# tiddoloos/Scaling-RGCN-training

Hardware: AMD Instinct MI355X
Metric: edges/s per RGCN layer (fwd+bwd) (higher is better)
Workload: dtype f32 (contraction: bf16x3 split of fp32 operands, fp32 accumulate)

## Files before the change

### include/rgcn_mi355x.h

```cpp
#ifndef RGCN_MI355X_H
#define RGCN_MI355X_H

#include <stddef.h>
#include <stdint.h>

#ifdef __cplusplus
extern "C" {
#endif

#define RGCN_ABI_VERSION 19
#define RGCN_UNIT 64
#define RGCN_CHUNK_MAX 128
#define RGCN_MAX_WIDTH 128
#define RGCN_XWIDE_MAX_WIDTH 512
#define RGCN_DW_WALKERS 2048

enum rgcn_act { RGCN_ACT_NONE = 0, RGCN_ACT_RELU = 1, RGCN_ACT_SIGMOID = 2 };

#define RGCN_FLAG_POINTER_GATHER 1u
#define RGCN_FLAG_DW_RING 2u
#define RGCN_FLAG_DW_DIRECT 4u
#define RGCN_FLAG_DW_ROOT_ONLY 16u
#define RGCN_FLAG_SPLIT_PRODUCERS 32u
#define RGCN_FLAG_EXACT_FP32 8u

enum rgcn_status {
    RGCN_OK = 0,
    RGCN_ERR_NULL = -1,
    RGCN_ERR_WIDTH = -2,
    RGCN_ERR_STRIDE = -3,
    RGCN_ERR_PLAN = -4,
    RGCN_ERR_LDS = -5,
    RGCN_ERR_WORKSPACE = -6,
    RGCN_ERR_DEVICE = -7,
    RGCN_ERR_ACT = -8,
    RGCN_ERR_GRAPH = -9,
    RGCN_ERR_ADDRESS = -10
};

typedef struct rgcn_plan {
    int32_t n_nodes;
    int32_t n_owned;
    int32_t num_relations;
    int32_t tile;
    int32_t n_tiles;
    int32_t n_chunks;
    int32_t chunk;
    int32_t n_units;
    int32_t layout;
    int32_t chunk_rows;
    const int32_t* tile_ptr;
    const int32_t* chunk_rel;
    const int32_t* chunk_cnt;
    const int32_t* chunk_tile;
    const int32_t* chunk_flags;
    const int32_t* rel_order;
    const int32_t* slot_src;
    const float* slot_w;
    const int32_t* slot_row;
    const int32_t* slot_acc;
    const int32_t* slot_src2;
} rgcn_plan_t;

int rgcn_abi_version(void);
const char* rgcn_status_string(int status);

typedef struct rgcn_graph {
    const int64_t* src;
    const int64_t* dst;
    const int64_t* type;
    int64_t src_stride, dst_stride, type_stride;
    int64_t num_edges;
    int32_t num_nodes;
    int32_t num_relations;
} rgcn_graph_t;

typedef struct rgcn_plan_sizes {
    int32_t n_tiles;
    int32_t n_chunks;
    int32_t n_units;
    int32_t reserved;
    int64_t n_slots;
    int64_t n_edges;
    uint64_t opaque[16];
} rgcn_plan_sizes_t;

size_t rgcn_plan_workspace_bytes(int64_t num_edges, int32_t n_owned, int32_t num_relations, int32_t tile);

int rgcn_edge_weights(const rgcn_graph_t* graph, int aggr_sum, float* w, void* workspace, size_t workspace_bytes, void* stream);

int rgcn_plan_build_begin(const rgcn_graph_t* graph, const float* w, int transposed, int32_t node_begin, int32_t node_end,
                          int32_t tile, int32_t chunk, int32_t layout, void* workspace, size_t workspace_bytes,
                          rgcn_plan_sizes_t* sizes, void* stream);
int rgcn_plan_build_finish(const rgcn_plan_sizes_t* sizes, void* workspace, size_t workspace_bytes, rgcn_plan_t* plan,
                           void* stream);

int rgcn_padded_width(int width);

size_t rgcn_packed_weight_floats(int num_relations, int din, int dout);

int rgcn_pack_weights(const float* weight, const float* root, int num_relations, int din, int dout,
                      int transpose, float* packed, void* stream);
int rgcn_pack_weights_basis(const float* bases, const float* comp, const float* root, int num_relations, int num_bases,
                            int din, int dout, int transpose, float* packed, void* stream);
int rgcn_pack_weights_block(const float* blocks, const float* root, int num_relations, int num_blocks, int din, int dout,
                            int transpose, float* packed, void* stream);
int rgcn_basis_backward(const float* d_w, const float* bases, const float* comp, int num_relations, int num_bases, int din,
// ... 81 lines not shown
```

### scaling_rgcn_training_amd/_lib.py

```python
from __future__ import annotations

import ctypes as C
import os
from typing import Optional

import torch

_HERE = os.path.dirname(os.path.abspath(__file__))
LIB_PATH = os.environ.get("RGCN_LIB") or os.path.join(_HERE, "librgcn_mi355x.so")
ABI_VERSION = 19

XWIDE_MAX_WIDTH = 512

ACT_NONE, ACT_RELU, ACT_SIGMOID = 0, 1, 2
ERR_PLAN = -4
ERR_ADDRESS = -10
FLAG_POINTER_GATHER, FLAG_DW_RING, FLAG_DW_DIRECT, FLAG_EXACT_FP32, FLAG_DW_ROOT_ONLY, FLAG_SPLIT_PRODUCERS = 1, 2, 4, 8, 16, 32


class RgcnPlanStruct(C.Structure):
    _fields_ = [
        ("n_nodes", C.c_int32), ("n_owned", C.c_int32), ("num_relations", C.c_int32),
        ("tile", C.c_int32), ("n_tiles", C.c_int32), ("n_chunks", C.c_int32), ("chunk", C.c_int32), ("n_units", C.c_int32),
        ("layout", C.c_int32), ("chunk_rows", C.c_int32),
        ("tile_ptr", C.c_void_p), ("chunk_rel", C.c_void_p), ("chunk_cnt", C.c_void_p),
        ("chunk_tile", C.c_void_p), ("chunk_flags", C.c_void_p), ("rel_order", C.c_void_p), ("slot_src", C.c_void_p),
        ("slot_w", C.c_void_p), ("slot_row", C.c_void_p), ("slot_acc", C.c_void_p), ("slot_src2", C.c_void_p),
    ]


class RgcnEdgeUnits(C.Structure):
    _fields_ = [("n_nodes", C.c_int32), ("n_units", C.c_int32), ("num_relations", C.c_int32), ("reserved", C.c_int32),
                ("unit_rel", C.c_void_p), ("unit_cnt", C.c_void_p), ("slot_src", C.c_void_p), ("slot_w", C.c_void_p)]


class RgcnGraphStruct(C.Structure):
    _fields_ = [("src", C.c_void_p), ("dst", C.c_void_p), ("type", C.c_void_p),
                ("src_stride", C.c_int64), ("dst_stride", C.c_int64), ("type_stride", C.c_int64),
                ("num_edges", C.c_int64), ("num_nodes", C.c_int32), ("num_relations", C.c_int32)]


class RgcnPlanSizes(C.Structure):
    _fields_ = [("n_tiles", C.c_int32), ("n_chunks", C.c_int32), ("n_units", C.c_int32), ("reserved", C.c_int32),
                ("n_slots", C.c_int64), ("n_edges", C.c_int64), ("opaque", C.c_uint64 * 16)]


def _prototypes() -> dict:
    vp, i32, u32, i64, sz, lng = C.c_void_p, C.c_int, C.c_uint, C.c_int64, C.c_size_t, C.c_long
    plan, units, graph, sizes, pint = (C.POINTER(RgcnPlanStruct), C.POINTER(RgcnEdgeUnits), C.POINTER(RgcnGraphStruct),
                                       C.POINTER(RgcnPlanSizes), C.POINTER(C.c_int))
    return {
        "rgcn_abi_version": (i32, []),
        "rgcn_status_string": (C.c_char_p, [i32]),
        "rgcn_padded_width": (i32, [i32]),
        "rgcn_packed_weight_floats": (sz, [i32, i32, i32]),
        "rgcn_pack_weights": (i32, [vp, vp, i32, i32, i32, i32, vp, vp]),
        "rgcn_fwd": (i32, [plan, vp, i32, i32, vp, vp, vp, i32, i32, i32, u32, vp]),
        "rgcn_bwd_dx": (i32, [plan, vp, i32, i32, vp, vp, i32, i32, vp, i32, u32, vp]),
        "rgcn_act_backward": (i32, [vp, vp, vp, lng, i32, i32, vp]),
        "rgcn_bwd_dw_workspace_bytes": (sz, [plan, i32, i32]),
        "rgcn_bwd_dw": (i32, [plan, vp, i32, i32, vp, i32, i32, vp, sz, vp, vp, vp, u32, vp]),
        "rgcn_plan_workspace_bytes": (sz, [i64, i32, i32, i32]),
        "rgcn_edge_weights": (i32, [graph, i32, vp, vp, sz, vp]),
        "rgcn_plan_build_begin": (i32, [graph, vp, i32, i32, i32, i32, i32, i32, vp, sz, sizes, vp]),
        "rgcn_plan_build_finish": (i32, [sizes, vp, sz, plan, vp]),
        "rgcn_dw_tiles_geometry": (i32, [pint, pint, pint]),
        "rgcn_dw_tiles_walk": (i32, [plan, vp, vp]),
        "rgcn_bwd_dw_tiles_workspace_bytes": (sz, [i32]),
        "rgcn_bwd_dw_tiles": (i32, [plan, vp, vp, i32, i32, vp, i32, i32, vp, sz, vp, u32, vp]),
        "rgcn_bwd_dw_root_workspace_bytes": (sz, []),
        "rgcn_bwd_dw_root": (i32, [vp, i32, i32, vp, i32, i32, lng, vp, sz, vp, vp, vp]),
        "rgcn_pack_weights_basis": (i32, [vp, vp, vp, i32, i32, i32, i32, i32, vp, vp]),
        "rgcn_pack_weights_block": (i32, [vp, vp, i32, i32, i32, i32, i32, vp, vp]),
        "rgcn_basis_backward": (i32, [vp, vp, vp, i32, i32, i32, i32, vp, vp, vp]),
        "rgcn_block_backward": (i32, [vp, i32, i32, i32, i32, vp, vp]),
        "rgcn_eplan_segments": (i32, [vp, i64, i32, vp, sz, vp, vp, vp]),
        "rgcn_ep_transform": (i32, [units, vp, i32, i32, vp, vp, i32, i32, u32, vp]),
        "rgcn_ep_segment_sum": (i32, [vp, i32, vp, vp, vp, i32, i32, vp, i32, vp, i32, i32, vp, i32, vp]),
        "rgcn_featureless_geometry": (i32, [i32, i32, i32, pint, pint]),
        "rgcn_featureless_fwd": (i32, [plan, vp, i64, vp, vp, i32, vp, vp, vp, i32, i32, vp]),
        "rgcn_featureless_bwd_workspace_bytes": (sz, [plan, i32, i32, i32]),
        "rgcn_featureless_bwd": (i32, [plan, vp, vp, vp, i64, vp, i32, i32, vp, vp, i32, vp, sz, vp, vp, vp, vp, vp]),
        "rgcn_xwide_geometry": (i32, [i32, i32, i32, pint, pint]),
        "rgcn_xwide_fwd": (i32, [plan, vp, i32, i32, vp, vp, vp, i32, i32, i32, vp]),
        "rgcn_xwide_bwd_dx": (i32, [plan, vp, i32, i32, vp, vp, i32, i32, vp, i32, vp]),
        "rgcn_xwide_bwd_dw_workspace_bytes": (sz, [plan, i32, i32]),
        "rgcn_xwide_bwd_dw": (i32, [plan, vp, i32, i32, vp, i32, i32, vp, sz, vp, vp, vp, vp]),
        "rgcn_segment_max": (i32, [vp, vp, i32, vp, vp, vp, i32, i32, vp, vp, i32, vp]),
        "rgcn_segment_max_bwd": (i32, [vp, i32, vp, vp, i32, vp, i32, vp, vp, vp, vp, i64, i32, vp, i32, vp]),
        "rgcn_rows_transform": (i32, [vp, i32, i32, vp, i32, vp, i32, vp, vp, i32, i32, lng, vp]),
        "rgcn_rows_dw_workspace_bytes": (sz, [i32, i32]),
        "rgcn_rows_dw": (i32, [vp, i32, i32, vp, i32, i32, lng, vp, sz, vp, vp]),
    }


_PROTOTYPES = _prototypes()
EXPORTS = tuple(_PROTOTYPES)


class RgcnLibraryError(RuntimeError):
# ... 472 lines not shown
```

### scaling_rgcn_training_amd/conv.py

```python
from __future__ import annotations

import math
import os
from collections import namedtuple
from typing import Optional, Tuple

import torch
from torch import Tensor, nn

from . import _lib
from .plan import GraphPlans, TilePlan, build_graph_plans, cached_graph_plans, choose_layout, padded_width


def _round4(n: int) -> int:
    return (n + 3) // 4 * 4


def _rows16(t: Tensor, width: int) -> Tensor:
    t = t.detach()
    if t.dtype != torch.float32:
        t = t.float()
    if width % 4 != 0:
        return torch.nn.functional.pad(t, (0, _round4(width) - width))
    return t.contiguous()
# ... 634 lines not shown
    if comp is not None:
        num_rel, dout = int(comp.shape[0]), int(weight.shape[2])
    elif weight.dim() == 4:
        num_rel, dout = int(weight.shape[0]), int(weight.shape[1] * weight.shape[3])
    else:
        num_rel, dout = int(weight.shape[0]), int(weight.shape[2])
    if xwide:
        if dctx is not None:
            raise NotImplementedError("RGCNConv wider than 128 runs on one GPU: a dist context is not supported")
        return _XwideFn.apply(x, weight, comp, root, bias, plans, act, bool(input_relu), premasked, num_relations or num_rel,
                              out_channels or dout)
    return _RGCNLayerFn.apply(x, weight, comp, root, bias, plans, dctx, act, bool(input_relu), premasked, int(flags),
                              num_relations or num_rel, out_channels or dout)


def _paths(path):
    return path if path == "auto" else ((path, path) if isinstance(path, str) else tuple(path))


_Route = namedtuple("_Route", "tile chunk layout dw_tiles split_producers paths")


def glorot_(t: Tensor) -> Tensor:
    bound = math.sqrt(6.0 / (t.size(-2) + t.size(-1)))
    with torch.no_grad():
        return t.uniform_(-bound, bound)


class RGCNConv(nn.Module):

    def __init__(self, in_channels: int, out_channels: int, num_relations: int,
                 num_bases: Optional[int] = None, num_blocks: Optional[int] = None, aggr: str = "mean",
                 root_weight: bool = True, is_sorted: bool = False, bias: bool = True, featureless: bool = False,
                 wide: Optional[bool] = None, **kwargs):
        super().__init__()
        if num_bases is not None and num_blocks is not None:
            raise ValueError("Can not apply both basis-decomposition and block-diagonal-decomposition "
                             "at the same time.")
        self.featureless = bool(featureless)
        if self.featureless and wide:
            raise ValueError("featureless RGCNConv has no wide mode: its tables stay at 1..128 columns")
        self.wide = (_WIDE_DEFAULT if wide is None else bool(wide)) and not self.featureless
        if self.featureless:
            if num_blocks is not None:
                raise ValueError("Block-diagonal decomposition not supported for non-continuous input features.")
            if isinstance(in_channels, (tuple, list)) or int(in_channels) != in_channels or in_channels < 1:
                raise ValueError(f"featureless RGCNConv: in_channels is the number of table rows, got {in_channels!r}")
            if not 1 <= out_channels <= 128:
                raise ValueError(f"RGCNConv out_channels must be in 1..128, got {out_channels}")
        in_channels_r = in_channels
        if isinstance(in_channels, (tuple, list)):
            if len(in_channels) != 2:
                raise ValueError(f"in_channels must be an int or a (source, destination) pair, got {in_channels!r}")
            in_channels, in_channels_r = int(in_channels[0]), int(in_channels[1])
        if aggr not in ("mean", "sum", "add", "max"):
            raise ValueError(f"unsupported aggr {aggr!r} (mean / sum / max)")
        if in_channels_r != in_channels:
            if aggr == "max":
                raise NotImplementedError("bipartite RGCNConv aggregates by mean / sum only: aggr='max' is not built")
            if self.wide and max(in_channels, in_channels_r, out_channels) > NARROW_MAX_WIDTH:
                raise NotImplementedError(f"bipartite RGCNConv takes 1..{NARROW_MAX_WIDTH} features per side, got "
                                          f"({in_channels}, {in_channels_r})->{out_channels} (wide layers are homogeneous)")
            if not 1 <= in_channels_r <= NARROW_MAX_WIDTH:
                raise ValueError(f"RGCNConv widths must be in 1..{NARROW_MAX_WIDTH}, got ({in_channels}, {in_channels_r})->{out_channels}")
        if aggr == "max" and self.featureless:
            raise ValueError("featureless RGCNConv has no max aggregation: aggr='max' takes float features x")
        if aggr == "max" and self.wide and max(in_channels, out_channels) > NARROW_MAX_WIDTH:
            raise NotImplementedError(f"RGCNConv(aggr='max') takes 1..{NARROW_MAX_WIDTH} features per side, got "
                                      f"{in_channels}->{out_channels} (wide layers aggregate by mean / sum only)")
        self.in_channels = in_channels
        self.in_channels_l = in_channels
        self.in_channels_r = in_channels_r
        self.out_channels = out_channels
        self.num_relations = num_relations
        self.num_bases = num_bases
        self.num_blocks = num_blocks
        self.aggr = "sum" if aggr == "add" else aggr
        self.is_sorted = is_sorted
        self.dist: Optional[DistContext] = None
        self._dist_plans = None
        self.kernel_flags = 0
        self.dw_tiles = True
        self.split_producers = _SPLIT_PRODUCERS_DEFAULT == "1"
        self.path = _PATH_DEFAULT
        self.merge_runs = _MERGE_RUNS_DEFAULT
        if num_bases is not None:
            self.weight = nn.Parameter(torch.empty(num_bases, in_channels, out_channels))
            self.comp = nn.Parameter(torch.empty(num_relations, num_bases))
        elif num_blocks is not None:
            assert in_channels % num_blocks == 0 and out_channels % num_blocks == 0, \
                "in_channels and out_channels must be divisible by num_blocks"
            self.weight = nn.Parameter(torch.empty(num_relations, num_blocks, in_channels // num_blocks,
                                                   out_channels // num_blocks))
            self.register_parameter("comp", None)
        else:
            self.weight = nn.Parameter(torch.empty(num_relations, in_channels, out_channels))
            self.register_parameter("comp", None)
        if root_weight:
            self.root = nn.Parameter(torch.empty(in_channels_r, out_channels))
        else:
            self.register_parameter("root", None)
        if bias:
            self.bias = nn.Parameter(torch.empty(out_channels))
        else:
            self.register_parameter("bias", None)
        if self.wide:
            if not (1 <= in_channels <= _lib.XWIDE_MAX_WIDTH and 1 <= out_channels <= _lib.XWIDE_MAX_WIDTH):
                raise ValueError(f"wide RGCNConv widths must be in 1..{_lib.XWIDE_MAX_WIDTH}, got {in_channels}->{out_channels}")
        elif not self.featureless:
            tile_for(in_channels, out_channels)
        self.reset_parameters()

    def reset_parameters(self) -> None:
        glorot_(self.weight)
        if self.comp is not None:
            glorot_(self.comp)
        if self.root is not None:
            glorot_(self.root)
        if self.bias is not None:
            with torch.no_grad():
                self.bias.zero_()

    def effective_weight(self) -> Tensor:
        if self.num_bases is not None:
            return (self.comp @ self.weight.view(self.num_bases, -1)).view(
                self.num_relations, self.in_channels, self.out_channels)
        if self.num_blocks is not None:
            nb = self.num_blocks
            bi, bo = self.in_channels // nb, self.out_channels // nb
            eye = torch.eye(nb, device=self.weight.device, dtype=self.weight.dtype)
            w = torch.einsum("rbio,bc->rbico", self.weight, eye)
            return w.reshape(self.num_relations, self.in_channels, self.out_channels)
        return self.weight

    def _plans(self, x: Tensor, edge_index: Tensor, edge_type: Tensor, route: Optional["_Route"] = None):
        n = x.shape[0]
        r = self._route(n, int(edge_type.shape[0]), x.is_cuda) if route is None else route
        widths = (self.in_channels, self.out_channels)
        if self.dist is None:
            return cached_graph_plans(edge_index, edge_type, n, self.num_relations, r.tile, self.aggr, chunk=r.chunk, split=r.layout,
                                      dw_tiles=r.dw_tiles, paths=r.paths, widths=widths)
        from .dist import cached_rank_plans
        return cached_rank_plans(edge_index, edge_type, n, self.num_relations, r.tile, self.aggr, self.dist, r.chunk, r.layout,
                                 r.dw_tiles, paths=r.paths, widths=widths)

    @property
    def _w64(self) -> bool:
        return padded_width(self.in_channels) == 64 and padded_width(self.out_channels) == 64

    def _use_split_producers(self, chunk: int) -> bool:
        return self.split_producers and chunk in (112, 128) and self._w64

    @property
    def xwide(self) -> bool:
        return self.wide and max(self.in_channels, self.out_channels) > NARROW_MAX_WIDTH

    def _route(self, n_nodes: int, n_edges: int, on_gpu: bool, plain: bool = False) -> "_Route":
        if self.xwide:
            raise NotImplementedError("RGCNConv wider than 128 runs on one GPU only: no dist layout")
        if self.aggr == "max":
            raise NotImplementedError("RGCNConv(aggr='max') runs on one GPU only: a dist context is not supported")
        tile, chunk = layout_for(self.in_channels, self.out_channels, n_nodes, n_edges, self.num_relations)
        dw_rule = self.dw_tiles and not plain and self._w64 and self.num_relations <= 32 and n_edges >= DW_TILES_MIN_EDGES
        exact_merge = False
        if self._use_split_producers(128):
            args = (n_nodes, n_edges, self.num_relations, self.in_channels, self.out_channels)
            t3, c3, cost3 = choose_layout(*args, kernel="bf16x3", with_cost=True)
            if cost3 <= choose_layout(*args, with_cost=True)[2]:
                tile, chunk = t3, c3
            elif chunk == 128:
                tile = min(tile, SPLIT_PRODUCERS_TILE)
        else:
            exact_merge = self.merge_runs and chunk == 128 and self._w64
            if exact_merge and dw_rule and self.kernel_flags == 0:
                tile = min(tile, EXACT_MERGE_TILE)
        split = self._use_split_producers(chunk)
        dw_tiles = (dw_rule and on_gpu and _lib.buffer_addressable(n_nodes, _round4(self.in_channels))
                    and _lib.buffer_addressable(n_nodes, _round4(self.out_channels)))
        layout = 3 if self.merge_runs and dw_tiles and self.kernel_flags == 0 and (split or exact_merge) else 0
        return _Route(tile, chunk, layout, dw_tiles, split, _paths(self.path) if on_gpu else ("ring", "ring"))

    def layout(self, n_nodes: int, n_edges: int) -> Tuple[int, int]:
        if self.aggr == "max":
            raise NotImplementedError("RGCNConv(aggr='max') has no tile layout: it runs on its own edge-parallel plan (eplan.MaxPlan)")
        r = self._route(n_nodes, n_edges, False)
        return r.tile, r.chunk

    def forward(self, x: Tensor, edge_index: Tensor, edge_type: Optional[Tensor] = None, *,
                _activation: Optional[str] = None, _input_relu: bool = False,
                _grad_premasked: bool = False) -> Tensor:
        assert edge_type is not None, "edge_type is required (PyG RGCNConv asserts the same)"
        if isinstance(x, (tuple, list)):
            return self._forward_bipartite(x, edge_index, edge_type, _activation, _input_relu, _grad_premasked)
        if self.featureless:
            return self._forward_featureless(x, edge_index, edge_type)
        if self.in_channels_r != self.in_channels:
            raise ValueError(f"this RGCNConv was built with in_channels=({self.in_channels}, {self.in_channels_r}): "
                             f"x must be a (x_src, x_dst) pair")
        if x is None or not torch.is_floating_point(x):
            raise NotImplementedError("featureless (integer / None x) RGCNConv is never used by the reference "
                                      "(x is always float: model/layers.py:21,62,108) and is not built")
        if x.dim() != 2 or x.shape[1] != self.in_channels:
            raise ValueError(f"x must be [N, {self.in_channels}], got {tuple(x.shape)}")
        if self.aggr == "max":
            return self._forward_max(x, edge_index, edge_type, _activation, _input_relu, _grad_premasked)
        if self.xwide:
            return self._forward_xwide(x, edge_index, edge_type, _activation, _input_relu, _grad_premasked)
        route = self._route(x.shape[0], int(edge_type.shape[0]), x.is_cuda)
        plans = self._plans(x, edge_index, edge_type, route)
        flags = self.kernel_flags | (_lib.FLAG_SPLIT_PRODUCERS if route.split_producers else 0)
        return rgcn_conv_function(x, self.weight, self.root, self.bias, plans, self.dist, _activation, _input_relu, _grad_premasked, flags,
                                  comp=self.comp, num_relations=self.num_relations, out_channels=self.out_channels)

    def _forward_xwide(self, x: Tensor, edge_index: Tensor, edge_type: Tensor, activation: Optional[str], input_relu: bool,
                       grad_premasked: bool) -> Tensor:
        if self.dist is not None:
            raise NotImplementedError("RGCNConv wider than 128 runs on one GPU: a dist context is not supported")
        paths = _paths(self.path)
        if paths != "auto" and "ep" in paths:
            raise ValueError("RGCNConv wider than 128 has no edge-parallel path: path must be 'auto' or 'ring'")
        _require_gpu(x)
        n = int(x.shape[0])
        tile, chunk = _lib.xwide_geometry(max(n, 1), self.in_channels, self.out_channels)
        plans = cached_graph_plans(edge_index, edge_type, n, self.num_relations, tile, self.aggr, chunk=chunk, extra_key=("xwide",))
        return rgcn_conv_function(x, self.weight, self.root, self.bias, plans, None, activation, input_relu, grad_premasked, 0,
                                  comp=self.comp, num_relations=self.num_relations, out_channels=self.out_channels, xwide=True)

    def _forward_max(self, x: Tensor, edge_index: Tensor, edge_type: Tensor, activation: Optional[str], input_relu: bool,
                     grad_premasked: bool) -> Tensor:
        if self.dist is not None:
            raise NotImplementedError("RGCNConv(aggr='max') runs on one GPU: a dist context is not supported")
        _require_gpu(x)
        if edge_index.device != x.device or edge_type.device != x.device:
            raise RuntimeError(f"RGCNConv(aggr='max'): edge_index ({edge_index.device}) and edge_type ({edge_type.device}) must be on "
                               f"the device of x ({x.device})")
        act, premasked = _fused(activation, grad_premasked)
        _lib.load()
        from .eplan import build_max_plan
        n, r = int(x.shape[0]), self.num_relations
        mp = cached_graph_plans(edge_index, edge_type, n, r, 0, "max", paths=("ep", "ep"), extra_key=("max",),
                                builder=lambda paths: build_max_plan(edge_index, edge_type, n, r))
        flags = self.kernel_flags | (_lib.FLAG_SPLIT_PRODUCERS if self.split_producers and self._w64 else 0)
        return _MaxLayerFn.apply(x, self.weight, self.comp, self.root, self.bias, mp, act, bool(input_relu), premasked, int(flags), r,
                                 self.out_channels)

    def _forward_bipartite(self, x, edge_index: Tensor, edge_type: Tensor, activation: Optional[str], input_relu: bool,
                           grad_premasked: bool) -> Tensor:
        if self.featureless:
            raise NotImplementedError("featureless RGCNConv takes x = None or node indices: a (x_src, x_dst) pair is not built")
        if self.aggr == "max":
            raise NotImplementedError("bipartite RGCNConv aggregates by mean / sum only: aggr='max' is not built")
        if self.xwide:
            raise NotImplementedError(f"bipartite RGCNConv takes 1..{NARROW_MAX_WIDTH} features per side (wide layers are homogeneous)")
        if self.dist is not None:
            raise NotImplementedError("bipartite RGCNConv runs on one GPU: a dist context is not supported")
        if activation is not None or input_relu or grad_premasked:
            raise ValueError("bipartite RGCNConv fuses no activation: _activation / _input_relu / _grad_premasked must be unset")
        if len(x) != 2:
            raise ValueError(f"x must be a (x_src, x_dst) pair, got {len(x)} members")
        x_src, x_dst = x
        for t in (x_src, x_dst):
            if not isinstance(t, Tensor) or not torch.is_floating_point(t):
                raise NotImplementedError("bipartite RGCNConv takes float features on both sides (no None / integer member)")
        if x_src.dim() != 2 or x_src.shape[1] != self.in_channels:
            raise ValueError(f"x_src must be [N_src, {self.in_channels}], got {tuple(x_src.shape)}")
        if x_dst.dim() != 2 or x_dst.shape[1] != self.in_channels_r:
            raise ValueError(f"x_dst must be [N_dst, {self.in_channels_r}], got {tuple(x_dst.shape)}")
        if x_src.dtype != torch.float32 or x_dst.dtype != torch.float32:
            raise ValueError(f"x_src and x_dst must be float32, got {x_src.dtype} and {x_dst.dtype}")
        if edge_index.dim() != 2 or edge_index.shape[0] != 2 or edge_type.dim() != 1 or edge_index.shape[1] != edge_type.shape[0]:
            raise ValueError(f"edge_index must be [2, E] and edge_type [E], got {tuple(edge_index.shape)} and {tuple(edge_type.shape)}")
        _require_gpu(x_src, x_dst)
        dev = x_src.device
        if x_dst.device != dev or edge_index.device != dev or edge_type.device != dev:
            raise RuntimeError(f"bipartite RGCNConv: x_dst ({x_dst.device}), edge_index ({edge_index.device}) and edge_type "
                               f"({edge_type.device}) must be on the device of x_src ({dev})")
        _lib.load()
        n_src, n_dst, e, r = int(x_src.shape[0]), int(x_dst.shape[0]), int(edge_type.shape[0]), self.num_relations
        n = max(n_src, n_dst)
        if e and min(n_src, n_dst) == 0:
            raise ValueError(f"edge_index out of range: {e} edges between {n_src} source and {n_dst} destination nodes")
        plans, flags = None, self.kernel_flags
        if n_dst > 0:
            route = self._route(n, e, True, plain=True)
            plans = self._bipartite_plans(edge_index, edge_type, n_src, n_dst, route)
            flags |= _lib.FLAG_SPLIT_PRODUCERS if route.split_producers else 0
        return _BipartiteFn.apply(x_src, x_dst, self.weight, self.comp, self.root, self.bias, plans, int(flags), r, self.out_channels)

    def _bipartite_plans(self, edge_index: Tensor, edge_type: Tensor, n_src: int, n_dst: int,
                         route: Optional["_Route"] = None) -> GraphPlans:
        e, r = int(edge_type.shape[0]), self.num_relations
        n = max(n_src, n_dst)
        route = self._route(n, e, True, plain=True) if route is None else route
# ... 37 lines not shown
```

### scaling_rgcn_training_amd/csrc/rgcn_tile3p.hip

```cpp
#include <type_traits>
#include "rgcn_common.h"
#include "rgcn_tile_common.h"

namespace rgcn {

constexpr int kP3Lookahead = 1;
constexpr int kP3PrioProducers = 0, kP3PrioConsumers = 3;

constexpr int kP3Threads = 512;
constexpr int kP3CH = 128;
template <int ST>
struct P3Geo {
    static constexpr int kPlaneBytes = 16 * ST * 128;
    static constexpr int kSlotBytes = 3 * kPlaneBytes;
};
constexpr int kP3LDO = kAccStride<64>;
constexpr int kP3FragsPerRel = 2 * 3 * 2 * 2;

__device__ __forceinline__ unsigned p3_cvt_pk_bf16(float lo, float hi) {
    unsigned r;
    asm("v_cvt_pk_bf16_f32 %0, %1, %2" : "=v"(r) : "v"(lo), "v"(hi));
    return r;
}

struct P3Rows {
    f32x4 v[8];
    int meta;
    int idx;
};

__device__ __forceinline__ void p3_load_rows(f32x4& dst, i32x4 rsrc, unsigned voff) {
    asm volatile("buffer_load_dwordx4 %0, %1, %2, 0 offen" : "=v"(dst) : "v"(voff), "s"(rsrc) : "memory");
}
__device__ __forceinline__ void p3_load_int(int& dst, const int* p) {
    asm volatile("global_load_dword %0, %1, off" : "=v"(dst) : "v"(p) : "memory");
}
template <int N>
__device__ __forceinline__ void p3_wait_batch(P3Rows& r) {
    asm volatile("s_waitcnt vmcnt(%10)"
                 : "+v"(r.v[0]), "+v"(r.v[1]), "+v"(r.v[2]), "+v"(r.v[3]), "+v"(r.v[4]), "+v"(r.v[5]), "+v"(r.v[6]), "+v"(r.v[7]),
                   "+v"(r.meta), "+v"(r.idx)
                 : "n"(N)
                 : "memory");
}

template <int ST>
__device__ __forceinline__ void p3_producer_loop(const TileArgs& a, char* ring, float* wring, int* dring, int c0, int nch,
                                                 int lane, int pw, int tile0) {
    constexpr int kP3PlaneBytes = P3Geo<ST>::kPlaneBytes, kP3SlotBytes = P3Geo<ST>::kSlotBytes, kP3SlotTiles = ST;
    int tile_cur = tile0;
    int tend = ldc(a.tile_ptr, tile0 + 1) - c0;
    auto tile_boundary = [&](int it) {
        if (it + 1 == tend && it + 1 < nch) {
            ++tile_cur;
            tend = ldc(a.tile_ptr, tile_cur + 1) - c0;
            wg_barrier();
        }
    };
    const int c = lane & 15, rq = lane >> 4;
    const unsigned long long xb = (unsigned long long)a.x;
    i32x4 rsrc;
    rsrc[0] = __builtin_amdgcn_readfirstlane((int)(unsigned)xb);
    rsrc[1] = __builtin_amdgcn_readfirstlane((int)((xb >> 32) & 0xFFFFull));
    rsrc[2] = __builtin_amdgcn_readfirstlane((int)a.x_bytes);
    rsrc[3] = 0x00020000;
    const unsigned coff = c < a.din4 ? (unsigned)c * 16u : 0xFFFFFFF0u;
    const unsigned rowb = c < a.din4 ? (unsigned)a.ldx * 4u : 0u;
    auto idx_ptr = [&](int k) {
        const int kk = k < nch ? k : nch - 1;
        return a.slot_src + (size_t)(c0 + kk) * kP3CH + 16 * ((lane & 31) >> 2) + 4 * pw + (lane & 3);
    };
    auto issue_loads = [&](P3Rows& r, int idxv) {
        int idx[8];
#pragma unroll
        for (int i = 0; i < 8; ++i) idx[i] = __builtin_amdgcn_ds_bpermute((4 * i + rq) * 4, idxv);
#pragma unroll
        for (int i = 0; i < 8; ++i) p3_load_rows(r.v[i], rsrc, __umul24((unsigned)idx[i], rowb) + coff);
    };
    const int mrow = 16 * ((lane & 31) >> 2) + 4 * pw + (lane & 3);
    const int half = pw & 1;
    const int* meta_src = a.merged ? (lane < 32 ? (const int*)a.slot_w : a.slot_acc) + mrow
                                   : (pw < 2 ? (const int*)a.slot_w : a.slot_acc) + 64 * half + lane;
    int* meta_dst = a.merged ? (int*)wring + 2 * mrow + (lane >> 5) : (int*)wring + 2 * (64 * half + lane) + (pw < 2 ? 0 : 1);
    auto issue_meta = [&](P3Rows& r, int k) { p3_load_int(r.meta, meta_src + (size_t)(c0 + k) * kP3CH); };
    auto store_meta = [&](const P3Rows& r, int k) { meta_dst[(k & 1) * 2 * kP3CH] = r.meta; };
    auto split_store = [&](P3Rows& r, int k, int nrt, int fl) {
        char* slot = ring + (k & 1) * kP3SlotBytes;
        if (fl & (7 << 16)) {
            const int ns1 = (fl >> 16) & 3;
            const bool ns2 = ((fl >> 18) & 1) != 0, pre = ((fl >> 19) & 1) != 0;
            if (pre) {
                auto wt = [&](int t) { return __int_as_float(__builtin_amdgcn_ds_bpermute((32 + 4 * t + rq) * 4, r.meta)); };
                r.v[0] += r.v[7] * wt(7);
                if (ns2) r.v[0] += ns1 >= 2 ? r.v[5] * wt(5) : r.v[6] * wt(6);
                if (ns1 >= 2) r.v[1] += r.v[6] * wt(6);
            } else {
                r.v[0] += r.v[7];
                if (ns2) r.v[0] += ns1 >= 2 ? r.v[5] : r.v[6];
                if (ns1 >= 2) r.v[1] += r.v[6];
            }
        }
#pragma unroll
        for (int i = 0; i < 8; ++i) {
            if (i >= nrt) break;
            const int row = 16 * i + 4 * pw + rq;
            const f32x4 vi = r.v[i];
            float x0 = vi[0], x1 = vi[1], x2 = vi[2], x3 = vi[3];
            unsigned h0, h1, m0, m1, l0, l1;
            split3_pair(x0, x1, h0, m0, l0);
            split3_pair(x2, x3, h1, m1, l1);
            char* p = slot + row * 128 + (((c >> 1) ^ ((row >> 1) & 7)) << 4) + ((c & 1) << 3);
            *(uint2*)p = make_uint2(h0, h1);
            *(uint2*)(p + kP3PlaneBytes) = make_uint2(m0, m1);
            *(uint2*)(p + 2 * kP3PlaneBytes) = make_uint2(l0, l1);
        }
    };
    auto issue_batch = [&](P3Rows& r, int j, int idx_rows) {
        issue_loads(r, idx_rows);
        issue_meta(r, j < nch ? j : nch - 1);
        p3_load_int(r.idx, idx_ptr(j + 2));
    };
    P3Rows r0, r1, r2;
    auto clear = [&](P3Rows& r) {
#pragma unroll
        for (int i = 0; i < 8; ++i) r.v[i] = f32x4{0.f, 0.f, 0.f, 0.f};
        r.meta = r.idx = 0;
    };
    clear(r0); clear(r1); clear(r2);
    p3_load_int(r1.idx, idx_ptr(0));
    p3_load_int(r2.idx, idx_ptr(1));
    p3_wait_batch<0>(r1);
    p3_wait_batch<0>(r2);
    const int i0 = r1.idx, i1 = r2.idx;
    issue_batch(r0, 0, i0);
    issue_batch(r1, 1, i1);
    p3_wait_batch<10>(r0);
    issue_batch(r2, 2, r0.idx);
    auto word_of = [&](int k) { return ldc(a.merged ? a.chunk_flags : a.chunk_cnt, c0 + (k < nch ? k : nch - 1)); };
    auto tiles_in = [&](int wd) { return min(kP3SlotTiles, a.merged ? (wd >> 20) & 15 : (wd + 15) >> 4); };
    auto flags_in = [&](int wd) { return a.merged ? wd : 0; };
    int wd_next = word_of(1);
    {
        const int wd0 = word_of(0);
        split_store(r0, 0, tiles_in(wd0), flags_in(wd0));
    }
    store_meta(r0, 0);
    wg_barrier();
    auto step = [&](int it, P3Rows& tgt, P3Rows& src) {
        p3_wait_batch<10>(src);
        __builtin_amdgcn_sched_barrier(0);
        if (it + 1 < nch) issue_batch(tgt, it + 3, src.idx);
        __builtin_amdgcn_sched_barrier(0);
        const int wd_now = wd_next;
        wd_next = word_of(it + 2);
        if (it + 1 < nch) {
            split_store(src, it + 1, tiles_in(wd_now), flags_in(wd_now));
            store_meta(src, it + 1);
        }
        __builtin_amdgcn_sched_barrier(0);
        wg_barrier();
        tile_boundary(it);
    };
    for (int it = 0; it < nch; it += 3) {
        step(it, r0, r1);
        if (it + 1 < nch) step(it + 1, r1, r2);
        if (it + 2 < nch) step(it + 2, r2, r0);
    }
    wait_vmcnt<0>();
}

template <int ST>
__global__ void __launch_bounds__(kP3Threads, 2) rgcn_tile3p_kernel(const TileArgs a) {
    constexpr int kP3PlaneBytes = P3Geo<ST>::kPlaneBytes, kP3SlotBytes = P3Geo<ST>::kSlotBytes, kP3SlotTiles = ST;
    constexpr int LDO = kP3LDO;
    extern __shared__ __attribute__((aligned(16))) float lds[];
    float* out_lds = lds;
    char* ring = (char*)(lds + (a.tile + 1) * LDO);
    float* wring = (float*)(ring + 2 * kP3SlotBytes);
    int* dring = (int*)(wring + 2 * kP3CH);

    const int tid = threadIdx.x;
    const int lane = tid & 63;
    const int wave = __builtin_amdgcn_readfirstlane(tid >> 6);
    const int tile0 = blockIdx.x * a.tiles_per_wg;
    const int tile1 = min(tile0 + a.tiles_per_wg, a.n_tiles);
    const int c0 = ldc(a.tile_ptr, tile0);
    const int nch = ldc(a.tile_ptr, tile1) - c0;

    tile_init<LDO>(a, out_lds, tid, kP3Threads);

    const bool is_consumer = wave >= 4;
    const int role_idx = wave >= 4 ? wave - 4 : wave;
    if (is_consumer) __builtin_amdgcn_s_setprio(kP3PrioConsumers);
    else __builtin_amdgcn_s_setprio(kP3PrioProducers);
    if (is_consumer) {
        const int cw = role_idx, cg = cw % 4;
        const int rowl = lane & 15, kq = lane >> 4;
        const unsigned col4_bytes = (unsigned)(16 * cg + 4 * kq) * 4u;
        const unsigned col1_bytes = (unsigned)(16 * cg + rowl) * 4u;
        const int wc = cg >> 1, wct0 = cg & 1;
        const uint4* wp4 = (const uint4*)a.wp + (size_t)(wc * 3 * 2 * 2 + wct0 * 2) * 64 + lane;
        auto wptr = [&](int rel, int pl) { return (const f32x4*)(wp4 + ((size_t)rel * kP3FragsPerRel + pl * 4) * 64); };
        f32x4 wcur[3][2], wnext[3][2];
        int rel_cur = ldc(a.chunk_rel, c0);
#pragma unroll
        for (int pl = 0; pl < 3; ++pl) {
            wcur[pl][0] = wptr(rel_cur, pl)[0];
            wcur[pl][1] = wptr(rel_cur, pl)[64];
        }
        __builtin_amdgcn_s_waitcnt(0x0F70);
        const i32x4 rs_cnt = make_srsrc(a.chunk_cnt + c0 + 1, 4L * (a.n_chunks - c0 - 1));
        const i32x4 rs_flg = make_srsrc(a.chunk_flags + c0 + 1, 4L * (a.n_chunks - c0 - 1));
        const i32x4 rs_rel = make_srsrc(a.chunk_rel + c0 + 3, 4L * (a.n_chunks - c0 - 3));
        unsigned moff = 0;
        int ld_cnt = ldc(a.chunk_cnt, c0);
        int ld_flg = ldc(a.chunk_flags, c0);
        int rel_n1 = nch > 1 ? ldc(a.chunk_rel, c0 + 1) : rel_cur;
        int ld_rel = nch > 2 ? ldc(a.chunk_rel, c0 + 2) : rel_n1;
        auto prefetch_rel = [&](int rel) {
#pragma unroll
            for (int pl = 0; pl < 3; ++pl) {
                prefetch16<0>(wnext[pl][0], wptr(rel, pl));
                prefetch16<1024>(wnext[pl][1], wptr(rel, pl));
            }
        };
        bool pending = rel_n1 != rel_cur;
        if (pending) prefetch_rel(rel_n1);
        int tile_cur = tile0;
        int tend = ldc(a.tile_ptr, tile0 + 1) - c0;
        wg_barrier();
        for (int it = 0; it < nch; ++it) {
            const int chunk = c0 + it;
            const int buf = it & 1;
            const int cnt = ld_cnt;
            const int flags_all = ld_flg;
            const int rel_next = rel_n1;
            const int rel_next2 = ld_rel;
            rel_n1 = ld_rel;
            sbuf_load(ld_cnt, rs_cnt, moff);
            sbuf_load(ld_flg, rs_flg, moff);
            sbuf_load(ld_rel, rs_rel, moff);
            moff += 4;
            (void)chunk;
            const bool swap_b = pending;
            const int nrt = min(kP3SlotTiles, (cnt + 15) >> 4);
            const int flags = flags_all & ((1 << nrt) - 1);
            const char* xrow[2];
#pragma unroll
            for (int s = 0; s < 2; ++s)
                xrow[s] = ring + buf * kP3SlotBytes + rowl * 128 + (((4 * s + kq) ^ ((rowl >> 1) & 7)) << 4);
            const int2* mb = (const int2*)wring + buf * kP3CH;
            struct Ops {
                bf16x8 pl[3][2];
                float w1;
                int d1;
            };
            auto load_ops = [&](Ops& o, int t) {
                const int2 wd = mb[t * 16 + rowl];
                o.w1 = __int_as_float(wd.x);
                o.d1 = wd.y;
#pragma unroll
                for (int pl = 0; pl < 3; ++pl)
#pragma unroll
                    for (int s = 0; s < 2; ++s) o.pl[pl][s] = *(const bf16x8*)(xrow[s] + pl * kP3PlaneBytes + t * 2048);
            };
            auto acc_ptr = [&](int d, unsigned col_bytes) -> float* {
                return (float*)((char*)out_lds + (__umul24((unsigned)d, (unsigned)(LDO * 4)) + col_bytes));
            };
            constexpr int px[6] = {0, 0, 1, 0, 2, 1}, pwl[6] = {0, 1, 0, 2, 0, 1};
            auto mfma_half = [&](const Ops& o, f32x4 y, int s) {
#pragma unroll
                for (int q = 0; q < 6; ++q)
                    y = __builtin_amdgcn_mfma_f32_16x16x32_bf16(__builtin_bit_cast(bf16x8, wcur[pwl[q]][s]), o.pl[px[q]][s], y, 0, 0, 0);
                return y;
            };
            auto consume = [&](auto nrt_c) {
                constexpr int NRT = decltype(nrt_c)::value;
                constexpr int LA = kP3Lookahead;
                Ops o[NRT];
                f32x4 y[NRT], old[NRT];
                float* dst[NRT];
#pragma unroll
                for (int t = 0; t < LA; ++t)
                    if (t < NRT) load_ops(o[t], t);
                __builtin_amdgcn_sched_barrier(0);
#pragma unroll
                for (int step = 0; step <= NRT; ++step) {
                    if (step < NRT) {
                        if (step + LA < NRT) load_ops(o[step + LA], step + LA);
                        y[step] = mfma_half(o[step], f32x4{0.f, 0.f, 0.f, 0.f}, 0);
                        __builtin_amdgcn_sched_barrier(0);
                    }
                    if (step >= 1) *(f32x4*)dst[step - 1] = y[step - 1] * o[step - 1].w1 + old[step - 1];
                    if (step < NRT) {
                        dst[step] = acc_ptr(o[step].d1, col4_bytes);
                        old[step] = *(const f32x4*)dst[step];
                    }
                    if (step < NRT) {
                        __builtin_amdgcn_sched_barrier(0);
                        y[step] = mfma_half(o[step], y[step], 1);
                        __builtin_amdgcn_sched_barrier(0);
                    }
                }
            };
            auto process_slow = [&](int t, bool dup) {
                Ops o;
                load_ops(o, t);
                if (!dup) {
                    float* d = acc_ptr(o.d1, col4_bytes);
                    const f32x4 oldv = *(const f32x4*)d;
                    f32x4 yv = mfma_half(o, f32x4{0.f, 0.f, 0.f, 0.f}, 0);
                    yv = mfma_half(o, yv, 1);
                    *(f32x4*)d = yv * o.w1 + oldv;
                    return;
                }
                f32x4 w4;
                i32x4 d4;
#pragma unroll
                for (int i = 0; i < 4; ++i) {
                    const int2 wd = mb[t * 16 + 4 * kq + i];
                    w4[i] = __int_as_float(wd.x);
                    d4[i] = wd.y;
                }
                float pm[4];
#pragma unroll
                for (int i = 0; i < 4; ++i) pm[i] = ((unsigned)d4[i] >> 24) == (unsigned)rowl ? w4[i] : 0.f;
                f32x4 yv = {0.f, 0.f, 0.f, 0.f};
#pragma unroll
                for (int s = 0; s < 2; ++s)
#pragma unroll
                    for (int q = 0; q < 6; ++q)
                        yv = __builtin_amdgcn_mfma_f32_16x16x32_bf16(o.pl[px[q]][s], __builtin_bit_cast(bf16x8, wcur[pwl[q]][s]), yv, 0, 0, 0);
                float* d[4];
                f32x4 oldv;
#pragma unroll
                for (int i = 0; i < 4; ++i) {
                    d[i] = acc_ptr(d4[i], col1_bytes);
                    oldv[i] = *d[i];
                }
                f32x4 z1 = {0.f, 0.f, 0.f, 0.f};
                f32x4 z0 = __builtin_amdgcn_mfma_f32_16x16x4f32(pm[0], yv[0], oldv, 0, 0, 0);
                z1 = __builtin_amdgcn_mfma_f32_16x16x4f32(pm[1], yv[1], z1, 0, 0, 0);
                z0 = __builtin_amdgcn_mfma_f32_16x16x4f32(pm[2], yv[2], z0, 0, 0, 0);
                z1 = __builtin_amdgcn_mfma_f32_16x16x4f32(pm[3], yv[3], z1, 0, 0, 0);
                const f32x4 v = z0 + z1;
#pragma unroll
                for (int i = 0; i < 4; ++i) *d[i] = v[i];
            };
            using std::integral_constant;
            if (flags == 0) {
                switch (nrt) {
                    case 1: consume(integral_constant<int, 1>{}); break;
                    case 2: consume(integral_constant<int, 2>{}); break;
                    case 3: consume(integral_constant<int, 3>{}); break;
                    case 4: consume(integral_constant<int, 4>{}); break;
                    case 5: consume(integral_constant<int, 5>{}); break;
                    case 6: consume(integral_constant<int, 6>{}); break;
                    case 7: consume(integral_constant<int, 7>{}); break;
                    case 8: if constexpr (ST >= 8) consume(integral_constant<int, 8>{}); break;
                    default: break;
                }
            } else {
                for (int t = 0; t < nrt; ++t) process_slow(t, (flags >> t) & 1);
            }
            if (swap_b) {
                wait_vmcnt<0>();
#pragma unroll
                for (int pl = 0; pl < 3; ++pl) {
                    wcur[pl][0] = wnext[pl][0];
                    wcur[pl][1] = wnext[pl][1];
                }
            }
            rel_cur = rel_next;
            pending = it + 2 < nch && rel_next2 != rel_next;
            if (pending) prefetch_rel(rel_next2);
            wg_barrier();
            sbuf_wait(ld_cnt, ld_flg, ld_rel);
            if (it + 1 == tend && it + 1 < nch) {
                tile_epilogue<LDO, true>(a, out_lds, tile_cur, cw * 64 + lane, 256);
                ++tile_cur;
                tend = ldc(a.tile_ptr, tile_cur + 1) - c0;
                __builtin_amdgcn_s_waitcnt(0x0F70);
                wg_barrier();
            }
        }
        __builtin_amdgcn_s_waitcnt(0x0F70);
    }
    if (!is_consumer) p3_producer_loop<ST>(a, ring, wring, dring, c0, nch, lane, role_idx, tile0);
    tile_epilogue<LDO, false>(a, out_lds, tile1 - 1, tid, kP3Threads);
}

static size_t p3_lds_bytes(int tile, int st) {
    return sizeof(float) * (size_t)(tile + 1) * kP3LDO + 2 * (size_t)(3 * 16 * st * 128) + 2 * kP3CH * 8;
}

template <int ST>
static int launch_tile3p_as(const TileArgs& b, int nwg, size_t lds, hipStream_t stream) {
    static std::atomic<unsigned long long> done{0};
    int dev = 0;
    hipError_t e = hipGetDevice(&dev);
    if (e != hipSuccess) return (int)e;
    const unsigned long long bit = 1ull << (dev & 63);
    if (!(done.load(std::memory_order_acquire) & bit)) {
        e = hipFuncSetAttribute((const void*)rgcn_tile3p_kernel<ST>, hipFuncAttributeMaxDynamicSharedMemorySize, kLdsBytes);
        if (e != hipSuccess) return (int)e;
        done.fetch_or(bit, std::memory_order_release);
    }
    hipLaunchKernelGGL((rgcn_tile3p_kernel<ST>), dim3(nwg), dim3(kP3Threads), lds, stream, b);
    return (int)hipGetLastError();
}

int launch_tile3p(const TileArgs& a, int n_tiles, int chunk_rows, void* stream) {
    if (a.x_bytes == 0) return RGCN_ERR_PLAN;
    const int st = chunk_rows > 0 && chunk_rows <= 112 ? 7 : 8;
    const size_t lds = p3_lds_bytes(a.tile, st);
    if (lds > (size_t)kLdsBytes) return RGCN_ERR_LDS;
    TileArgs b = a;
    if (n_tiles < 16 * 256) b.tiles_per_wg = 1;
    const int nwg = (n_tiles + b.tiles_per_wg - 1) / b.tiles_per_wg;
    if (st == 7) return launch_tile3p_as<7>(b, nwg, lds, (hipStream_t)stream);
    return launch_tile3p_as<8>(b, nwg, lds, (hipStream_t)stream);
}

}
```

### scaling_rgcn_training_amd/csrc/rgcn_tile_fp32.hip

```cpp
#include "rgcn_kernels_shared.h"

namespace rgcn {

int dispatch_tile_narrow(int KP, int NP, const TileArgs& a, int n_tiles, int chunk, void* stream);
int dispatch_tile_wide(int KP, int NP, const TileArgs& a, int n_tiles, int chunk, void* stream);

static int dispatch_tile(int KP, int NP, const TileArgs& a, int n_tiles, int chunk, hipStream_t s) {
    return KP <= 32 ? dispatch_tile_narrow(KP, NP, a, n_tiles, chunk, s) : dispatch_tile_wide(KP, NP, a, n_tiles, chunk, s);
}


static int run_tile(const rgcn_plan_t* plan, const float* x, int ldx, int kin, const float* packed, const float* bias,
                    float* out, int ldo, int nout, int act, const float* mask, int ldm, unsigned flags, void* stream) {
    int st = check_plan(plan);
    if (st != RGCN_OK) return st;
    if (plan->layout == 2) return RGCN_ERR_PLAN;
    if (plan->layout == 5) return RGCN_ERR_PLAN;
    if (!x || !packed || !out) return RGCN_ERR_NULL;
    if ((st = check_stride(ldx, kin)) != RGCN_OK) return st;
    if ((st = check_stride(ldo, nout)) != RGCN_OK) return st;
    if (mask != nullptr && (st = check_stride(ldm, nout)) != RGCN_OK) return st;
    if (act != RGCN_ACT_NONE && act != RGCN_ACT_RELU && act != RGCN_ACT_SIGMOID) return RGCN_ERR_ACT;
    if ((st = check_device()) != RGCN_OK) return st;
    TileArgs a;
    a.tile_ptr = plan->tile_ptr;
    a.chunk_rel = plan->chunk_rel;
    a.chunk_cnt = plan->chunk_cnt;
    a.chunk_flags = plan->chunk_flags;
    a.slot_src = plan->slot_src;
    a.slot_w = plan->slot_w;
    a.slot_acc = plan->slot_acc;
    a.x = x;
    a.wp = packed;
    a.bias = bias;
    a.out = out;
    a.ldx = ldx;
    a.x_bytes = buffer_bytes(plan->n_nodes, ldx, flags);
    a.n_rows = plan->n_nodes;
    a.din4 = (kin + 3) / 4;
    a.dout = nout;
    a.ldo = ldo;
    a.tile = plan->tile;
    a.n_owned = plan->n_owned;
    a.mask = mask;
    a.ldm = ldm;
    a.act = act;
    a.n_tiles = plan->n_tiles;
    a.n_chunks = plan->n_chunks;
    a.merged = plan->layout == 3 ? 1 : 0;
    a.tiles_per_wg = tiles_per_workgroup(plan->n_tiles);
    a.reserved = 0;
    const int KP = padded_width(kin), NP = padded_width(nout);
    if ((flags & RGCN_FLAG_SPLIT_PRODUCERS) && !(flags & RGCN_FLAG_EXACT_FP32) && KP == 64 && NP == 64 && plan->chunk == 128 &&
        a.x_bytes != 0) {
        TileArgs b = a;
        b.wp = packed + (size_t)(plan->num_relations + 1) * KP * NP;
        const int st3 = launch_tile3p(b, plan->n_tiles, plan->chunk_rows, stream);
        if (st3 != RGCN_ERR_LDS || plan->layout == 3) return st3;
    }
    if (plan->layout == 3 && !(KP == 64 && NP == 64 && plan->chunk == 128 && a.x_bytes != 0)) return RGCN_ERR_PLAN;
    return dispatch_tile(KP, NP, a, plan->n_tiles, plan->chunk, (hipStream_t)stream);
}

}

using namespace rgcn;


extern "C" int rgcn_fwd(const rgcn_plan_t* plan, const float* x, int ldx, int din, const float* packed_w,
                        const float* bias, float* out, int ldo, int dout, int act, unsigned flags, void* stream) {
    return run_tile(plan, x, ldx, din, packed_w, bias, out, ldo, dout, act, nullptr, 0, flags, stream);
}

extern "C" int rgcn_bwd_dx(const rgcn_plan_t* plan_t, const float* g, int ldg, int dout, const float* packed_wt,
                           float* dx, int lddx, int din, const float* relu_of, int ldr, unsigned flags, void* stream) {
    return run_tile(plan_t, g, ldg, dout, packed_wt, nullptr, dx, lddx, din, RGCN_ACT_NONE, relu_of, ldr, flags, stream);
}
```

Before: 4.425 billion.

## Fuse tile output stores into root-relation chunk consume in split-producer kernel

When the root relation is the last chunk processed for a tile, the consumer now applies the final update plus optional ReLU and writes results straight to global memory with buffer stores. It then resets the LDS accumulator to the bias, so the separate tile epilogue and its barriers are skipped. Producers also stop synchronising at tile boundaries in this mode. The aim is to remove the epilogue pass over LDS and its workgroup barriers. It assumes the root chunk comes last in each tile, and dropping those barriers risks races if that ordering does not hold.

```diff
diff --git a/include/rgcn_mi355x.h b/include/rgcn_mi355x.h
--- a/include/rgcn_mi355x.h
+++ b/include/rgcn_mi355x.h
@@ -23,6 +23,7 @@
 #define RGCN_FLAG_DW_ROOT_ONLY 16u
 #define RGCN_FLAG_SPLIT_PRODUCERS 32u
 #define RGCN_FLAG_EXACT_FP32 8u
+#define RGCN_FLAG_ROOT_STORES 64u
 
 enum rgcn_status {
     RGCN_OK = 0,
diff --git a/scaling_rgcn_training_amd/_lib.py b/scaling_rgcn_training_amd/_lib.py
--- a/scaling_rgcn_training_amd/_lib.py
+++ b/scaling_rgcn_training_amd/_lib.py
@@ -16,6 +16,7 @@
 ERR_PLAN = -4
 ERR_ADDRESS = -10
 FLAG_POINTER_GATHER, FLAG_DW_RING, FLAG_DW_DIRECT, FLAG_EXACT_FP32, FLAG_DW_ROOT_ONLY, FLAG_SPLIT_PRODUCERS = 1, 2, 4, 8, 16, 32
+FLAG_ROOT_STORES = 64
 
 
 class RgcnPlanStruct(C.Structure):
diff --git a/scaling_rgcn_training_amd/conv.py b/scaling_rgcn_training_amd/conv.py
--- a/scaling_rgcn_training_amd/conv.py
+++ b/scaling_rgcn_training_amd/conv.py
@@ -740,6 +740,7 @@
         self.kernel_flags = 0
         self.dw_tiles = True
         self.split_producers = _SPLIT_PRODUCERS_DEFAULT == "1"
+        self._root_stores = _lib.FLAG_ROOT_STORES
         self.path = _PATH_DEFAULT
         self.merge_runs = _MERGE_RUNS_DEFAULT
         if num_bases is not None:
@@ -866,7 +867,7 @@
             return self._forward_xwide(x, edge_index, edge_type, _activation, _input_relu, _grad_premasked)
         route = self._route(x.shape[0], int(edge_type.shape[0]), x.is_cuda)
         plans = self._plans(x, edge_index, edge_type, route)
-        flags = self.kernel_flags | (_lib.FLAG_SPLIT_PRODUCERS if route.split_producers else 0)
+        flags = self.kernel_flags | (_lib.FLAG_SPLIT_PRODUCERS | self._root_stores if route.split_producers else 0)
         return rgcn_conv_function(x, self.weight, self.root, self.bias, plans, self.dist, _activation, _input_relu, _grad_premasked, flags,
                                   comp=self.comp, num_relations=self.num_relations, out_channels=self.out_channels)
 
diff --git a/scaling_rgcn_training_amd/csrc/rgcn_tile3p.hip b/scaling_rgcn_training_amd/csrc/rgcn_tile3p.hip
--- a/scaling_rgcn_training_amd/csrc/rgcn_tile3p.hip
+++ b/scaling_rgcn_training_amd/csrc/rgcn_tile3p.hip
@@ -43,6 +43,11 @@
                  : "n"(N)
                  : "memory");
 }
+
+__device__ __forceinline__ void p3_store_piece(f32x4 v, i32x4 rsrc, unsigned voff) {
+    asm volatile("buffer_store_dwordx4 %0, %1, %2, 0 offen" ::"v"(v), "v"(voff), "s"(rsrc) : "memory");
+}
+constexpr unsigned kP3NoStore = 0x80000000u;
 
 template <int ST>
 __device__ __forceinline__ void p3_producer_loop(const TileArgs& a, char* ring, float* wring, int* dring, int c0, int nch,
@@ -54,7 +59,7 @@
         if (it + 1 == tend && it + 1 < nch) {
             ++tile_cur;
             tend = ldc(a.tile_ptr, tile_cur + 1) - c0;
-            wg_barrier();
+            if (a.reserved < 0) wg_barrier();
         }
     };
     const int c = lane & 15, rq = lane >> 4;
@@ -208,6 +213,22 @@
             wcur[pl][0] = wptr(rel_cur, pl)[0];
             wcur[pl][1] = wptr(rel_cur, pl)[64];
         }
+        const int root_rel = a.reserved;
+        const unsigned ldo_bytes = (unsigned)a.ldo * 4u;
+        const unsigned gcol = 4 * cg + kq < ((a.dout + 3) >> 2) ? col4_bytes : kP3NoStore;
+        f32x4 bfin = {0.f, 0.f, 0.f, 0.f};
+        if (root_rel >= 0 && a.bias != nullptr) {
+#pragma unroll
+            for (int c = 0; c < 4; ++c) bfin[c] = 16 * cg + 4 * kq + c < a.dout ? a.bias[16 * cg + 4 * kq + c] : 0.f;
+        }
+        i32x4 orsrc = {0, 0, 0, 0x00020000};
+        auto out_tile = [&](int t) {
+            const unsigned long long ob = (unsigned long long)a.out + (unsigned long long)t * (unsigned)a.tile * ldo_bytes;
+            orsrc[0] = __builtin_amdgcn_readfirstlane((int)(unsigned)ob);
+            orsrc[1] = __builtin_amdgcn_readfirstlane((int)((ob >> 32) & 0xFFFFull));
+            orsrc[2] = __builtin_amdgcn_readfirstlane((int)((unsigned)min(a.tile, a.n_owned - t * a.tile) * ldo_bytes));
+        };
+        if (root_rel >= 0) out_tile(tile0);
         __builtin_amdgcn_s_waitcnt(0x0F70);
         const i32x4 rs_cnt = make_srsrc(a.chunk_cnt + c0 + 1, 4L * (a.n_chunks - c0 - 1));
         const i32x4 rs_flg = make_srsrc(a.chunk_flags + c0 + 1, 4L * (a.n_chunks - c0 - 1));
@@ -242,7 +263,7 @@
             sbuf_load(ld_rel, rs_rel, moff);
             moff += 4;
             (void)chunk;
-            const bool swap_b = pending;
+            bool swap_b = pending;
             const int nrt = min(kP3SlotTiles, (cnt + 15) >> 4);
             const int flags = flags_all & ((1 << nrt) - 1);
             const char* xrow[2];
@@ -274,12 +295,14 @@
                     y = __builtin_amdgcn_mfma_f32_16x16x32_bf16(__builtin_bit_cast(bf16x8, wcur[pwl[q]][s]), o.pl[px[q]][s], y, 0, 0, 0);
                 return y;
             };
-            auto consume = [&](auto nrt_c) {
+            auto consume = [&](auto nrt_c, auto fin_c) {
                 constexpr int NRT = decltype(nrt_c)::value;
+                constexpr int FINAL = decltype(fin_c)::value;
                 constexpr int LA = kP3Lookahead;
                 Ops o[NRT];
                 f32x4 y[NRT], old[NRT];
                 float* dst[NRT];
+                unsigned goff[NRT];
 #pragma unroll
                 for (int t = 0; t < LA; ++t)
                     if (t < NRT) load_ops(o[t], t);
@@ -291,9 +314,22 @@
                         y[step] = mfma_half(o[step], f32x4{0.f, 0.f, 0.f, 0.f}, 0);
                         __builtin_amdgcn_sched_barrier(0);
                     }
-                    if (step >= 1) *(f32x4*)dst[step - 1] = y[step - 1] * o[step - 1].w1 + old[step - 1];
+                    if (step >= 1) {
+                        f32x4 v = y[step - 1] * o[step - 1].w1 + old[step - 1];
+                        if constexpr (FINAL != 0) {
+                            if constexpr (FINAL == 2) {
+#pragma unroll
+                                for (int c = 0; c < 4; ++c) v[c] = v[c] > 0.f ? v[c] : 0.f;
+                            }
+                            p3_store_piece(v, orsrc, goff[step - 1]);
+                            *(f32x4*)dst[step - 1] = bfin;
+                        } else {
+                            *(f32x4*)dst[step - 1] = v;
+                        }
+                    }
                     if (step < NRT) {
                         dst[step] = acc_ptr(o[step].d1, col4_bytes);
+                        if constexpr (FINAL != 0) goff[step] = __umul24((unsigned)o[step].d1, ldo_bytes) + gcol;
                         old[step] = *(const f32x4*)dst[step];
                     }
                     if (step < NRT) {
@@ -348,17 +384,34 @@
                 for (int i = 0; i < 4; ++i) *d[i] = v[i];
             };
             using std::integral_constant;
+            auto consume_nrt = [&](auto fin_c) {
+                switch (nrt) {
+                    case 1: consume(integral_constant<int, 1>{}, fin_c); break;
+                    case 2: consume(integral_constant<int, 2>{}, fin_c); break;
+                    case 3: consume(integral_constant<int, 3>{}, fin_c); break;
+                    case 4: consume(integral_constant<int, 4>{}, fin_c); break;
+                    case 5: consume(integral_constant<int, 5>{}, fin_c); break;
+                    case 6: consume(integral_constant<int, 6>{}, fin_c); break;
+                    case 7: consume(integral_constant<int, 7>{}, fin_c); break;
+                    case 8: if constexpr (ST >= 8) consume(integral_constant<int, 8>{}, fin_c); break;
+                    default: break;
+                }
+            };
             if (flags == 0) {
-                switch (nrt) {
-                    case 1: consume(integral_constant<int, 1>{}); break;
-                    case 2: consume(integral_constant<int, 2>{}); break;
-                    case 3: consume(integral_constant<int, 3>{}); break;
-                    case 4: consume(integral_constant<int, 4>{}); break;
-                    case 5: consume(integral_constant<int, 5>{}); break;
-                    case 6: consume(integral_constant<int, 6>{}); break;
-                    case 7: consume(integral_constant<int, 7>{}); break;
-                    case 8: if constexpr (ST >= 8) consume(integral_constant<int, 8>{}); break;
-                    default: break;
+                if (rel_cur != root_rel) {
+                    consume_nrt(integral_constant<int, 0>{});
+                } else {
+                    if (swap_b) wait_vmcnt<0>();
+                    if (a.act == RGCN_ACT_RELU) consume_nrt(integral_constant<int, 2>{});
+                    else consume_nrt(integral_constant<int, 1>{});
+                    if (swap_b) {
+#pragma unroll
+                        for (int pl = 0; pl < 3; ++pl) {
+                            wcur[pl][0] = wnext[pl][0];
+                            wcur[pl][1] = wnext[pl][1];
+                        }
+                        swap_b = false;
+                    }
                 }
             } else {
                 for (int t = 0; t < nrt; ++t) process_slow(t, (flags >> t) & 1);
@@ -377,17 +430,21 @@
             wg_barrier();
             sbuf_wait(ld_cnt, ld_flg, ld_rel);
             if (it + 1 == tend && it + 1 < nch) {
-                tile_epilogue<LDO, true>(a, out_lds, tile_cur, cw * 64 + lane, 256);
+                if (root_rel < 0) tile_epilogue<LDO, true>(a, out_lds, tile_cur, cw * 64 + lane, 256);
                 ++tile_cur;
                 tend = ldc(a.tile_ptr, tile_cur + 1) - c0;
-                __builtin_amdgcn_s_waitcnt(0x0F70);
-                wg_barrier();
+                if (root_rel < 0) {
+                    __builtin_amdgcn_s_waitcnt(0x0F70);
+                    wg_barrier();
+                } else {
+                    out_tile(tile_cur);
+                }
             }
         }
         __builtin_amdgcn_s_waitcnt(0x0F70);
     }
     if (!is_consumer) p3_producer_loop<ST>(a, ring, wring, dring, c0, nch, lane, role_idx, tile0);
-    tile_epilogue<LDO, false>(a, out_lds, tile1 - 1, tid, kP3Threads);
+    if (a.reserved < 0) tile_epilogue<LDO, false>(a, out_lds, tile1 - 1, tid, kP3Threads);
 }
 
 static size_t p3_lds_bytes(int tile, int st) {
diff --git a/scaling_rgcn_training_amd/csrc/rgcn_tile_fp32.hip b/scaling_rgcn_training_amd/csrc/rgcn_tile_fp32.hip
--- a/scaling_rgcn_training_amd/csrc/rgcn_tile_fp32.hip
+++ b/scaling_rgcn_training_amd/csrc/rgcn_tile_fp32.hip
@@ -49,12 +49,15 @@
     a.n_chunks = plan->n_chunks;
     a.merged = plan->layout == 3 ? 1 : 0;
     a.tiles_per_wg = tiles_per_workgroup(plan->n_tiles);
-    a.reserved = 0;
+    a.reserved = -1;
     const int KP = padded_width(kin), NP = padded_width(nout);
     if ((flags & RGCN_FLAG_SPLIT_PRODUCERS) && !(flags & RGCN_FLAG_EXACT_FP32) && KP == 64 && NP == 64 && plan->chunk == 128 &&
         a.x_bytes != 0) {
         TileArgs b = a;
         b.wp = packed + (size_t)(plan->num_relations + 1) * KP * NP;
+        if ((flags & RGCN_FLAG_ROOT_STORES) && mask == nullptr && (act == RGCN_ACT_NONE || act == RGCN_ACT_RELU) && ldo <= 4096 &&
+            (plan->layout == 0 || plan->layout == 1 || plan->layout == 3))
+            b.reserved = plan->num_relations;
         const int st3 = launch_tile3p(b, plan->n_tiles, plan->chunk_rows, stream);
         if (st3 != RGCN_ERR_LDS || plan->layout == 3) return st3;
     }
```

Result: slower. 4.309 billion (-2.6%).
